# UDC-GAC/pRIblast

Measured on AMD Instinct MI355X. Metric: query RNAs/sec in `ris` step, higher is better.
Workload: dtype f64

## Files before the change

priblast_amd/csrc/gapped_args.hpp:

```cpp
#pragma once
#include <hip/hip_runtime.h>

#include <cstdint>

#include "search_device.hpp"
#include "search_kernels.hpp"

namespace prb {

struct Rec32 {
  using word = uint32_t;
  static constexpr bool kBases = true;
  static __device__ __forceinline__ word pack(int i, int j, int pred, int type, int qa, int da) {
    return (word)i | ((word)j << 7) | ((word)pred << 14) | ((word)type << 21) | ((word)qa << 24) | ((word)da << 27);
  }
  static __device__ __forceinline__ int i(word v) { return v & 0x7F; }
  static __device__ __forceinline__ int j(word v) { return (v >> 7) & 0x7F; }
  static __device__ __forceinline__ int pred(word v) { return (v >> 14) & 0x7F; }
  static __device__ __forceinline__ int type(word v) { return (v >> 21) & 7; }
  static __device__ __forceinline__ int qa(word v) { return (v >> 24) & 7; }
  static __device__ __forceinline__ int da(word v) { return (v >> 27) & 7; }
};



struct DirOrigin {
  int q_start, id_start, id_end;
  int64_t db_start;
};
__device__ __forceinline__ DirOrigin dir_origin(const HitState &h, int flag) {
  DirOrigin o;
  if (flag == 0) {
    o.q_start = h.q_sp;
    o.db_start = h.db_sp;
  } else {
    o.q_start = h.q_sp + h.q_len - 1;
    o.db_start = (int64_t)h.db_sp + h.db_len - 1;
  }
  o.id_start = h.id_start;
  o.id_end = h.id_start + h.db_len - 1;
  return o;
}


struct GapArgs {
  HitSoA in, out;
  int64_t n;
  const uint32_t *subset;
  QBatchDev qb;
  PageDev pg;
  SearchConst sc;
  ExtOpts o;
  uint8_t *overflow;
  uint8_t *tier_out;
  int tier_id;
  const uint8_t *first_flag;
  int32_t *bp_count;
  uint16_t *trace;
  const int64_t *bp_off;
  int32_t *bp_out;
  unsigned long long *next_work;
  GapResume rin, rout;
  LongTrace lt;
  double *acc_scratch = nullptr;
  int period = 0;
  int early = 0;
  int handover = 0;
};


}
```

priblast_amd/csrc/gapped_lds.hip:

```cpp
#include <algorithm>
#include <type_traits>

#include "gapped_args.hpp"
#include "search_device.hpp"
#include "search_kernels.hpp"

namespace prb {

#ifdef PRB_GAP_PROFILE
constexpr int kProfSlots = 26;
__device__ unsigned long long g_gap_prof[10 * kProfSlots];
struct GapProf {
  unsigned long long last, acc[kProfSlots];
  int cells_now = 0, cells_prev = 0;
  __device__ __forceinline__ void start() {
    for (int i = 0; i < kProfSlots; i++) acc[i] = 0;
    last = __builtin_amdgcn_s_memtime();
  }
  __device__ __forceinline__ void mark(int r) {
    const unsigned long long t = __builtin_amdgcn_s_memtime();
    acc[r] += t - last;
    last = t;
  }
  __device__ __forceinline__ void count(int r) { acc[r] += 1; }
  __device__ __forceinline__ void flush(int kind) {
    if ((threadIdx.x & 63) == 0)
      for (int i = 0; i < kProfSlots; i++) atomicAdd(&g_gap_prof[kind * kProfSlots + i], acc[i]);
  }
};
#define GP_MARK(r) prof.mark(r)
#define GP_COUNT(r) prof.count(r)
#else
struct GapProf {
  __device__ __forceinline__ void start() {}
  __device__ __forceinline__ void flush(int) {}
};
#define GP_MARK(r)
#define GP_COUNT(r)
#endif

namespace {

constexpr int kInitStage = 16;
struct Tier0 {
#ifndef PRB_T0_CAPR
#define PRB_T0_CAPR 48
#define PRB_T0_WGCU 4
#endif
#ifndef PRB_T0_ACC_GLOBAL
#define PRB_T0_ACC_GLOBAL false
#endif
  static constexpr int kG = 8, kCapD = 32, kCapR = PRB_T0_CAPR, kGroups = 32, kWavesPerSimd = PRB_T0_WGCU, kWgPerCu = PRB_T0_WGCU;
  static constexpr bool kResumable = true;
  static constexpr bool kResumes = false;
  static constexpr bool kPairSteps = true;
  static constexpr bool kAccGlobal = PRB_T0_ACC_GLOBAL;
};
#ifndef PRB_T12_ACC_GLOBAL
#define PRB_T12_ACC_GLOBAL true
#endif
#ifndef PRB_T12_WPS
#define PRB_T12_WPS (PRB_T12_ACC_GLOBAL ? 4 : 3)
#endif
#ifndef PRB_T1_CAPD
#define PRB_T1_CAPD 40
#define PRB_T1_CAPR 64
#define PRB_T1_GROUPS 32
#define PRB_T1_WGCU (PRB_T12_ACC_GLOBAL ? 4 : 3)
#endif
struct Tier1 {
  static constexpr int kG = 8, kCapD = PRB_T1_CAPD, kCapR = PRB_T1_CAPR, kGroups = PRB_T1_GROUPS, kWavesPerSimd = PRB_T12_WPS, kWgPerCu = PRB_T1_WGCU;
  static constexpr bool kResumable = true, kResumes = true;
  using From = Tier0;
  using FromRec = Rec32;
  static constexpr bool kPairSteps = false;
  static constexpr bool kAccGlobal = PRB_T12_ACC_GLOBAL;
};
struct Tier2 {
  static constexpr int kG = 16, kCapD = 64, kCapR = 120, kGroups = 16, kWavesPerSimd = PRB_T12_WPS, kWgPerCu = PRB_T12_ACC_GLOBAL ? 4 : 3;
  static constexpr bool kResumable = true, kResumes = true;
  using From = Tier1;
  using FromRec = Rec32;
  static constexpr bool kPairSteps = false;
  static constexpr bool kAccGlobal = PRB_T12_ACC_GLOBAL;
};
struct Tier3 {
  static constexpr int kG = 64, kCapD = 128, kCapR = 512, kGroups = 1, kWavesPerSimd = 4, kWgPerCu = 16;
  static constexpr bool kResumable = false, kResumes = true;
  using From = Tier2;
  using FromRec = Rec32;
  static constexpr bool kPairSteps = false;
  static constexpr bool kAccGlobal = false;
};

struct Rec32W {
  using word = uint32_t;
  static constexpr bool kBases = false;
  static __device__ __forceinline__ word pack(int i, int j, int pred, int type, int, int) {
    return (word)i | ((word)j << 8) | ((word)pred << 16) | ((word)type << 25);
  }
  static __device__ __forceinline__ int i(word v) { return v & 0xFF; }
  static __device__ __forceinline__ int j(word v) { return (v >> 8) & 0xFF; }
  static __device__ __forceinline__ int pred(word v) { return (v >> 16) & 0x1FF; }
  static __device__ __forceinline__ int type(word v) { return (v >> 25) & 7; }
// ... 644 lines not shown
        w |= (uint32_t)dpp_i32<0x141>((int)w);
        tw[c] = w;
        cells |= (cells_t)((__ballot(type1 != 0) >> gbase) & 0xFF) << (8 * c);
        GP_COUNT(11);
      }
    }
    GP_MARK(3);
#ifdef PRB_GAP_PROFILE
    prof.cells_now = kChunks <= 4 ? __popc((uint32_t)cells) : __popcll((unsigned long long)cells);
#endif
    while (cells) {
      const cells_t rest = cells & (cells - 1);
      const bool two = rest != 0 && d.nrec + 2 <= S.cap_r();
      const int b0 = kChunks <= 4 ? __builtin_ctz((uint32_t)cells) : __builtin_ctzll((unsigned long long)cells);
      if (Store::kResumable && d.nrec >= S.cap_r()) {
        d.overflow = true;
        d.resume_i0 = i_lo + b0;
        d.resume_dstart = dstart;
        break;
      }
      int b = b0;
      if (two) {
        const int b1 = kChunks <= 4 ? __builtin_ctz((uint32_t)rest) : __builtin_ctzll((unsigned long long)rest);
        if (gl >= G / 2) b = b1;
        cells = rest & (rest - 1);
      } else {
        cells = rest;
      }
      uint32_t w = tw[0];
#pragma unroll
      for (int c = 1; c < kChunks; c++) w = (b >> 3) == c ? tw[c] : w;
      const int ptype = fill_cell(i_lo + b, (int)((w >> (3 * (b & 7))) & 7), two);
      if (ptype < 0) {
        d.overflow = true;
        break;
      }
    }
    group_sync<kLds>();
    GP_MARK(3);
  } else {
    for (int i0 = i_lo; i0 <= i_hi && !d.overflow; i0 += G) {
      const int type1 = cell_type(i0 + gl);
      using mask_t = typename std::conditional<G <= 32, uint32_t, unsigned long long>::type;
      const unsigned long long tb0 = __ballot(type1 & 1), tb1 = __ballot(type1 & 2), tb2 = __ballot(type1 & 4);
      const unsigned long long anyb = tb0 | tb1 | tb2;
      mask_t vmask = G < 64 ? (mask_t)((anyb >> gbase) & ((1ull << (G & 63)) - 1)) : (mask_t)anyb;
      GP_MARK(3);
      GP_COUNT(11);
      if (Store::kResumable && d.nrec + __popcll((unsigned long long)vmask) > S.cap_r()) {
        d.overflow = true;
        d.resume_i0 = i0;
        d.resume_dstart = dstart;
        break;
      }
      while (vmask) {
        if constexpr (G == 64) {
          const int left = __popcll((unsigned long long)vmask), n = left < 4 ? left : 4;
          if (n >= 2 && d.nrec + n <= S.cap_r()) {
            fill_quad(i0, (unsigned long long)vmask, n, tb0, tb1, tb2);
            for (int t = 0; t < n; t++) vmask &= vmask - 1;
            continue;
          }
        }
        const int b = G <= 32 ? __builtin_ctz((uint32_t)vmask) : __builtin_ctzll((unsigned long long)vmask);
        vmask &= vmask - 1;
        const int ctype = (int)((tb0 >> (gbase + b)) & 1) | (int)(((tb1 >> (gbase + b)) & 1) << 1) |
                          (int)(((tb2 >> (gbase + b)) & 1) << 2);
        const int ptype = fill_cell(i0 + b, ctype, false);
        if (ptype < 0) {
          d.overflow = true;
          break;
        }
      }
      group_sync<kLds>();
      GP_MARK(3);
    }
  }
  if (d.overflow) return true;
  if (d.length - (d.min_ci + d.min_cj) >= drop) return true;
  if (!q_open && !d_open) return true;
  return false;
}

template <class Store>
__device__ __forceinline__ bool dir_step_pair(const SearchConst &sc, const SeqBases &sb, const ExtOpts &o, const HitCtx &c, int flag,
                                              const Store &S, int gl, int gbase, DirState &d, GapProf &prof) {
  constexpr int G = 8;
  using R = typename Store::R;
  static_assert(Store::kCapD <= 32, "a 32-bit mask of cells per anti-diagonal");
  constexpr int kChunks = (Store::kCapD + G - 1) / G;
  const int delta = o.delta, drop = o.drop_w_gap, min_helix = o.min_helix;
  const bool mid = d.resume_i0 != 0;
  if (!mid) {
    if (d.length >= S.cap_d()) {
      d.overflow = true;
      return true;
    }
    d.length++;
  }
  const int LA = d.length;
  const bool openA = LA < d.tq0 || LA < d.td0;
  const int curA = LA - 3 * ((LA * 171) >> 9), d2A = curA == 2 ? 0 : curA + 1;
  if (!mid) {
    if (LA > d.staged) stage_acc_regs<G, true>(sb, c, flag, delta, S, gl, gbase, d, LA);
    GP_MARK(1);
    GP_COUNT(10);
    uint64_t *row = reinterpret_cast<uint64_t *>(&S.ptab(curA, 0));
    for (int t = gl; t < S.ptab_len() / 8; t += G) row[t] = 0;
    group_sync<true>();
    if (LA - 2 > drop) {
      while (d.lo < d.nrec) {
        const auto v = S.info(d.lo);
        if (LA - R::i(v) - R::j(v) - 2 > drop) d.lo++;
        else break;
      }
    }
  }
  GP_MARK(2);
  const int dstartA = mid ? d.resume_dstart : d.nrec, loA = d.lo;
  const int i_firstA = LA - d.td0 + 1 > 1 ? LA - d.td0 + 1 : 1;
  const int i_loA = mid ? d.resume_i0 : i_firstA;
  const int i_hiA = (LA < d.tq0 ? LA : d.tq0) - 1;
  d.resume_i0 = 0;

  auto pair_type = [&](int i, int j) -> int {
    const unsigned x0 = (unsigned)S.qb(i) * 5 + S.db(j);
    int t = (int)((sc.bp_rows >> ((x0 * 3 - 15) & 63)) & 7);
    if (flag == 1) t = ((t - 1) ^ 1) + 1;
    return t;
  };
  auto helix_ok = [&](unsigned x0, unsigned x1, unsigned x2, int pt, int i, int j) -> bool {
    const unsigned p0 = (sc.pair_mask >> x0) & 1, w0 = (sc.wobble_mask >> x0) & 1;
    unsigned ahead = 1;
    if (min_helix >= 2) ahead = ((sc.pair_mask >> x1) & 1) & ~(w0 & (sc.wobble_mask >> x1));
    if (min_helix >= 3) ahead &= sc.pair_mask >> x2;
    for (int x = 3; x <= min_helix - 1; x++) ahead &= sc.pair_mask >> ((unsigned)S.qb(i + x) * 5 + S.db(j + x));
    const unsigned need = (unsigned)(pt == 0) | (w0 & (unsigned)wobble(pt));
    return (p0 & (ahead | ~need) & 1) != 0;
  };

  const int LB = LA + 1, d2B = curA == 0 ? 2 : curA - 1;
  const bool try_pair = !mid && openA && LA - (d.min_ci + d.min_cj) < drop && LA < S.cap_d() && LB <= d.staged;
  uint32_t cellsA = 0, cellsB = 0;
  int loB = loA;
  bool paired = false;
  if (try_pair) {
    if (LB - 2 > drop) {
      while (loB < dstartA) {
        const auto v = S.info(loB);
        if (LB - R::i(v) - R::j(v) - 2 > drop) loB++;
        else break;
      }
    }
    const int i_loB = LB - d.td0 + 1 > 1 ? LB - d.td0 + 1 : 1, i_hiB = (LB < d.tq0 ? LB : d.tq0) - 1;
#pragma unroll
    for (int ch = 0; ch < kChunks; ch++) {
      const int i0 = i_loA + ch * G;
      if (i0 <= i_hiB) {
        const int i = i0 + gl, j = LA - i, jc = j < 0 ? 0 : j;
        const unsigned q0 = (unsigned)S.qb(i) * 5, q1 = (unsigned)S.qb(i + 1) * 5, q2 = (unsigned)S.qb(i + 2) * 5;
        const unsigned d0 = S.db(jc), d1 = S.db(jc + 1), d2b = S.db(jc + 2), d3 = S.db(jc + 3);
        const bool okA = i <= i_hiA && helix_ok(q0 + d0, q1 + d1, q2 + d2b, S.ptab(d2A, i - 1), i, j);
        const bool okB = i >= i_loB && i <= i_hiB && helix_ok(q0 + d1, q1 + d2b, q2 + d3, S.ptab(d2B, i - 1), i, j + 1);
        cellsA |= (uint32_t)((__ballot(okA) >> gbase) & 0xFF) << (8 * ch);
        cellsB |= (uint32_t)((__ballot(okB) >> gbase) & 0xFF) << (8 * ch);
        GP_COUNT(11);
      }
    }
    if (d.nrec + __popc(cellsA) + __popc(cellsB) <= S.cap_r()) {
      paired = true;
      uint64_t *row = reinterpret_cast<uint64_t *>(&S.ptab(d2A, 0));
      for (int t = gl; t < S.ptab_len() / 8; t += G) row[t] = 0;
      group_sync<true>();
      GP_COUNT(10);
    } else {
      cellsB = 0;
    }
  } else {
#pragma unroll
    for (int ch = 0; ch < kChunks; ch++) {
      const int i0 = i_loA + ch * G;
      if (i0 <= i_hiA) {
        const int i = i0 + gl, j = LA - i, jc = j < 0 ? 0 : j;
        const unsigned x0 = (unsigned)S.qb(i) * 5 + S.db(jc), x1 = (unsigned)S.qb(i + 1) * 5 + S.db(jc + 1),
                       x2 = (unsigned)S.qb(i + 2) * 5 + S.db(jc + 2);
        const bool okA = i <= i_hiA && helix_ok(x0, x1, x2, S.ptab(d2A, i - 1), i, j);
        cellsA |= (uint32_t)((__ballot(okA) >> gbase) & 0xFF) << (8 * ch);
        GP_COUNT(11);
      }
    }
  }
  const int nA = __popc(cellsA);
  int typeA0 = 0;
  if (paired && nA != 0) {
    const int iA0 = i_loA + __builtin_ctz(cellsA);
    typeA0 = rtype_of(pair_type(iA0, LA - iA0));
  }
#ifdef PRB_GAP_PROFILE
  prof.cells_now = nA + __popc(cellsB);
#endif
  GP_MARK(3);

  auto fill_cell = [&](int ci, bool isB, bool two) -> int {
    GP_COUNT(12);
    const bool pair_mode = two, hi = pair_mode && gl >= G / 2;
    const int sub = pair_mode ? (gl & (G / 2 - 1)) : gl, stride = pair_mode ? G / 2 : G;
    const int L = LA + (isB ? 1 : 0), cur = isB ? (curA == 2 ? 0 : curA + 1) : curA, lo = isB ? loB : loA;
    const int cj = L - ci;
    const int ctype = pair_type(ci, cj);
    const int nq = S.qb(ci - 1), nd = S.db(cj - 1);
    double bte = 1000000.0;
    int bkp = lo << 3;
    const typename R::word v0 = lo + sub < dstartA ? S.info(lo + sub) : 0;
    scan_qualifying<R>(
        S, lo, dstartA, sub, stride, ci, cj, v0,
        [&](typename R::word v) -> double {
          const int ri = R::i(v), rj = R::j(v);
          const int rq = R::qa(v), rd = R::da(v);
          const bool f0 = flag == 0;
          const int rt = R::type(v);
          return loop_energy_abcd(sc, f0 ? ctype : rt, f0 ? rt : ctype, ci - ri - 1, cj - rj - 1, f0 ? nq : rq, f0 ? nd : rd,
                                  f0 ? rq : nq, f0 ? rd : nd);
        },
        bte, bkp, prof);
    GP_MARK(4);
    group_min_halves(bte, bkp, pair_mode);
    GP_MARK(5);
    if (d.nrec >= S.cap_r()) return -1;
    int bk = bkp >> 3, ptype = bkp & 7;
    const bool a_first = isB && typeA0 != 0 && lo >= dstartA;
    if (lo >= dstartA && !a_first) bk = 0;
    if (ptype == 0) ptype = a_first ? typeA0 : R::type(S.info(bk));
    const int rec = d.nrec + (hi ? 1 : 0);
    if (sub == 0) {
      S.hyb(rec) = bte;
      S.info(rec) = R::pack(ci, cj, bk, rtype_of(ctype), S.qb(ci + 1), S.db(cj + 1));
      S.ptab(cur, ci) = (uint8_t)ptype;
    }
    const double ie = S.eq(ci - 1) + S.ed(cj - 1) + bte;
    const double ie_o = dpp_f64<0x141>(ie);
    const int ci_o = dpp_i32<0x141>(ci), cj_o = dpp_i32<0x141>(cj);
    const double ie_a = hi ? ie_o : ie, ie_b = hi ? ie : ie_o;
    const int ci_a = hi ? ci_o : ci, ci_b = hi ? ci : ci_o, cj_a = hi ? cj_o : cj, cj_b = hi ? cj : cj_o;
    if (ie_a < d.min_e) {
      d.min_e = ie_a;
      d.best = d.nrec;
      d.min_ci = ci_a;
      d.min_cj = cj_a;
    }
    if (pair_mode && ie_b < d.min_e) {
      d.min_e = ie_b;
      d.best = d.nrec + 1;
      d.min_ci = ci_b;
      d.min_cj = cj_b;
    }
    d.nrec += pair_mode ? 2 : 1;
    GP_MARK(6);
    return ptype;
  };

  unsigned long long cells = (unsigned long long)cellsA | ((unsigned long long)cellsB << 32);
  while (cells) {
    const unsigned long long rest = cells & (cells - 1);
    const bool two = rest != 0 && d.nrec + 2 <= S.cap_r();
    const int b0 = __builtin_ctzll(cells);
    if (Store::kResumable && d.nrec >= S.cap_r()) {
      d.overflow = true;
      d.resume_i0 = i_loA + b0;
      d.resume_dstart = dstartA;
      break;
    }
    int b = b0;
    if (two) {
      if (gl >= G / 2) b = __builtin_ctzll(rest);
      cells = rest & (rest - 1);
    } else {
      cells = rest;
    }
    const bool isB = b >= 32;
    const int ptype = fill_cell(i_loA + (b & 31), isB, two);
    if (ptype < 0) {
      d.overflow = true;
      break;
    }
  }
  group_sync<true>();
  GP_MARK(3);
  if (d.overflow) return true;
  if (paired) {
    d.length = LA + 1;
    d.lo = loB;
    if (LB - (d.min_ci + d.min_cj) >= drop) return true;
    return !(LB < d.tq0 || LB < d.td0);
  }
  if (LA - (d.min_ci + d.min_cj) >= drop) return true;
  return !openA;
}

template <class Store> __device__ __forceinline__ DirResult dir_finish(const DirState &d, HitState &h, int flag, const Store &S) {
  DirResult r;
  r.overflow = d.overflow;
  r.best = d.min_ci != 0 ? d.best : 0;
  if (d.min_ci != 0) {
    h.e_acc = h.e_acc + S.eq(d.min_ci - 1) + S.ed(d.min_cj - 1);
    if (flag == 0) {
      h.q_sp -= d.min_ci;
      h.db_sp -= d.min_cj;
    } else {
      h.id_start -= d.min_cj;
    }
    h.q_len += d.min_ci;
    h.db_len += d.min_cj;
  }
  h.e_tot = d.min_e;
  return r;
}

struct ResumeHeader {
  DirState d;
  double acc_prev1;
  HitState h;
  int32_t flag, nleft;
};
template <class T, class Rec> constexpr size_t resume_bytes() {
  return (sizeof(ResumeHeader) + sizeof(LdsState<T, Rec>) + 63) & ~(size_t)63;
}

template <int G, class T, class Rec>
__device__ __forceinline__ void resume_dump(const GapResume &ro, const HitCtx &c, const DirState &d, int flag,
                                            const LdsStore<T, Rec> &S, int gl, int gbase) {
  int slot = -1;
  if (gl == 0) {
    slot = (int)atomicAdd(ro.count, 1u);
    if (slot >= ro.cap) slot = -1;
  }
  slot = __shfl(slot, gbase);
  if (slot < 0) return;
  uint8_t *dst = ro.pool + (size_t)slot * resume_bytes<T, Rec>();
  ResumeHeader *H = reinterpret_cast<ResumeHeader *>(dst);
  if (gl == 0) {
    H->d = d;
    H->h = c.h;
    H->flag = flag;
    H->nleft = c.nleft;
    ro.slot[c.x] = slot;
  } else if (gl == 1) {
    H->acc_prev1 = d.acc_prev;
  }
  if constexpr (!T::kAccGlobal) {
    uint32_t *w = reinterpret_cast<uint32_t *>(dst + sizeof(ResumeHeader));
    const uint32_t *src = reinterpret_cast<const uint32_t *>(&S.s);
#pragma unroll 2
    for (int t = gl; t < (int)(sizeof(LdsState<T, Rec>) / 4); t += G) w[t] = src[t];
  } else {
    LdsState<T, Rec> *o = reinterpret_cast<LdsState<T, Rec> *>(dst + sizeof(ResumeHeader));
    for (int t = gl; t < T::kCapD; t += G) {
      o->eq[t] = S.eq(t);
      o->ed[t] = S.ed(t);
    }
    for (int t = gl; t < d.nrec; t += G) {
      o->hyb[t] = S.hyb(t);
      o->info[t] = S.info(t);
    }
    uint32_t *pw = reinterpret_cast<uint32_t *>(&o->ptab[0][0]);
    const uint32_t *ps = reinterpret_cast<const uint32_t *>(&S.s.ptab[0][0]);
    for (int t = gl; t < 3 * LdsState<T, Rec>::kPtabLen / 4; t += G) pw[t] = ps[t];
  }
}

template <int G, class TS, class RecS, class Store>
__device__ __forceinline__ void resume_load(const GapResume &ri, int slot, const GapArgs &a, HitCtx &c, DirState &d, int &flag,
                                            const Store &S, int gl) {
  using R = typename Store::R;
  const uint8_t *src = ri.pool + (size_t)slot * resume_bytes<TS, RecS>();
  const ResumeHeader *H = reinterpret_cast<const ResumeHeader *>(src);
  d = H->d;
  if (G > 1 && gl == 1) d.acc_prev = H->acc_prev1;
  d.overflow = false;
  c.h = H->h;
// ... 129 lines not shown
      a.bp_count[x] = c.nleft;
      a.tier_out[x] = (uint8_t)(kResumeMark | ((c.resumed ? c.tier0 : a.tier_id) & kMarkTier));
    }
    if (!c.ovf) {
      const int64_t x = c.x;
      int tcode = a.tier_id > c.tier0 ? a.tier_id : c.tier0;
      if (a.tier_id == kWaveTier && a.lt.slot) {
        const int ls = a.lt.slot[x];
        if (ls >= 0) {
          const int c0 = a.lt.count[ls * 2], c1 = a.lt.count[ls * 2 + 1];
          if ((c0 >= 0 || (c0 == -1 && c.nleft <= kTraceCap)) && c1 >= 0) tcode = kLongTraceTier;
        }
      }
      a.tier_out[x] = (uint8_t)tcode;
      a.bp_count[x] = c.nleft | (c.nright << 16);
      const double d0 = dangle_energy_gapped(sc, h.q_sp, h.db_sp, 0, qs, c.qn, ds, a.pg.nchars);
      const double d1 = dangle_energy_gapped(sc, h.q_sp + US(h.q_len) - 1, (int64_t)h.db_sp + US(h.db_len) - 1, 1, qs, c.qn,
                                             ds, a.pg.nchars);
      double e = h.e_tot, hy = h.e_tot - h.e_acc;
      e += d0;
      e += d1;
      hy += d0;
      hy += d1;
      a.out.q_sp[x] = h.q_sp;
      a.out.db_sp[x] = h.db_sp;
      a.out.q_len[x] = h.q_len;
      a.out.db_len[x] = h.db_len;
      a.out.db_id[x] = c.id;
      a.out.db_id_start[x] = h.id_start;
      a.out.query[x] = c.query;
      a.out.e_acc[x] = h.e_acc;
      a.out.e_hyb[x] = hy;
      a.out.e_tot[x] = e;
    }
  } else if (!c.ovf) {
    int t = 0;
    const int64_t d0 = c.unsorted ? c.out0 : c.out0 + c.nleft;
    for (int u = 0; u < c.diag_len; u++)
      if (diag_pairs(sc, qs[c.diag_q + u], ds[c.diag_d + u])) {
        a.bp_out[2 * (d0 + t)] = c.diag_q + u;
        a.bp_out[2 * (d0 + t) + 1] = c.diag_d + u;
        t++;
      }
  }
}

__device__ __forceinline__ void hit_handover(const GapArgs &a, int64_t w, const HitCtx &c, int gl) {
  if (gl != 0) return;
  const int64_t x = c.x;
  const HitState &h = c.h;
  a.overflow[w] = 0;
  a.out.q_sp[x] = h.q_sp;
  a.out.db_sp[x] = h.db_sp;
  a.out.q_len[x] = h.q_len;
  a.out.db_len[x] = h.db_len;
  a.out.db_id_start[x] = h.id_start;
  a.out.e_acc[x] = h.e_acc;
  a.out.e_hyb[x] = h.e_tot - h.e_acc;
  a.out.e_tot[x] = h.e_tot;
  a.bp_count[x] = c.nleft;
  a.tier_out[x] = (uint8_t)(kHandoverMark | (a.tier_id & kMarkTier));
}

__global__ __launch_bounds__(256) void k_bp_count(HitSoA in, int64_t n, const uint32_t *__restrict__ subset, QBatchDev qb,
                                                  PageDev pg, SearchConst sc, const int32_t *__restrict__ ntrace,
                                                  int32_t *bp_count) {
  const int64_t w = (int64_t)blockIdx.x * 256 + threadIdx.x;
  if (w >= n) return;
  const int64_t x = subset ? (int64_t)subset[w] : w;
  const uint8_t *qs = qb.enc + qb.off[in.query[x]] + in.q_sp[x];
  const uint8_t *ds = pg.seqs + in.db_sp[x];
  const int len = US(in.q_len[x]);
  int c = 0;
  for (int t = 0; t < len; t++) c += diag_pairs(sc, qs[t], ds[t]);
  bp_count[w] = c + (ntrace[x] & 0xFFFF) + (int)((uint32_t)ntrace[x] >> 16);
}

template <int kMode, class T, class Rec, bool kPair>
#ifdef PRB_TIERS_VGPR128
__global__ __launch_bounds__(T::kG *T::kGroups) __attribute__((amdgpu_num_vgpr(128))) void k_gapped_lds(GapArgs a) {
#else
__global__ __launch_bounds__(T::kG *T::kGroups, T::kWavesPerSimd) void k_gapped_lds(GapArgs a) {
#endif
  static_assert(!kPair || (T::kPairSteps && T::kG == 8), "dir_step_pair");
  __shared__ LdsLive<T, Rec> lds[T::kGroups];
  constexpr int G = T::kG;
  const int gl = threadIdx.x & (G - 1);
  const int gbase = (threadIdx.x & 63) & ~(G - 1);
  const int gid = threadIdx.x / G;
  const LdsStore<T, Rec> S{lds[gid], T::kAccGlobal ? a.acc_scratch + ((size_t)blockIdx.x * T::kGroups + gid) * 2 * T::kCapD : nullptr};
  const int64_t ngroups = (int64_t)gridDim.x * T::kGroups;
  GapProf prof;
  prof.start();
  int64_t w = (int64_t)blockIdx.x * T::kGroups + gid;
  enum { kLoad, kInit, kRun, kFinished, kDone };
  int phase = w < a.n ? kLoad : kDone, flag = 0;
  const int period = a.period > 0 ? a.period : kPair ? (a.o.drop_w_gap > 1 ? (a.o.drop_w_gap + 1) / 2 : 1) : (a.o.drop_w_gap > 1 ? a.o.drop_w_gap : 1);
  int tick = 0;
  HitCtx c;
  DirState d;
  const SeqBases sb{a.qb.enc, a.qb.acc, a.qb.cond, a.pg.acc, a.pg.cond};
  while (__ballot(phase != kDone) != 0) {
    GP_MARK(14);
    if (a.early > 0 && tick != 0 && __popcll(__ballot(phase == kFinished)) >= a.early * G) tick = 0;
    if (tick == 0) {
      if (phase == kFinished) {
        DirResult r{true, 0};
        const DirOrigin og = dir_origin(c.h, flag);
        if (!d.overflow) {
          r = dir_finish(d, c.h, flag, S);
        } else {
          if constexpr (kMode == 0 && T::kResumable)
            if (a.rout.slot) resume_dump<G, T, Rec>(a.rout, c, d, flag, S, gl, gbase);
        }
        hit_dir_done<kMode, true>(a, c, flag, og, r, S, gl);
        group_sync<true>();
        GP_MARK(7);
        const bool hand = kMode == 0 && a.handover && !c.ovf && flag == 0 && !c.resumed;
        if (c.ovf || flag == 1 || hand) {
          if (hand) hit_handover(a, w, c, gl);
          else hit_store<kMode>(a, w, c, flag, gl);
          unsigned long long nw = 0;
          if (gl == 0) nw = (unsigned long long)ngroups + atomicAdd(a.next_work, 1ull);
          w = (int64_t)__shfl(nw, gbase);
          phase = w < a.n ? kLoad : kDone;
          GP_MARK(9);
        } else {
          flag = 1;
          phase = kInit;
        }
      }
      if (phase == kLoad) {
        hit_load<kMode>(a, w, c);
        flag = c.resumed ? 1 : 0;
        phase = kInit;
        if constexpr (kMode == 0 && T::kResumes) {
          const int slot = a.rin.slot ? a.rin.slot[c.x] : -1;
          if (slot >= 0) {
            resume_load<G, typename T::From, typename T::FromRec>(a.rin, slot, a, c, d, flag, S, gl);
            phase = kRun;
          }
        }
        GP_MARK(8);
      }
      if (phase == kInit) {
        dir_init<G, true>(a.sc, sb, c, flag, a.pg.seqs, a.pg.nchars, S, gl, a.o.delta, d);
        phase = kRun;
        GP_MARK(0);
      }
    }
    GP_MARK(15);
#ifdef PRB_GAP_PROFILE
    prof.cells_now = 0;
#endif
    if constexpr (kPair) {
      if (phase == kRun && dir_step_pair(a.sc, sb, a.o, c, flag, S, gl, gbase, d, prof)) phase = kFinished;
    } else {
      if (phase == kRun && dir_step<G, true>(a.sc, sb, a.o, c, flag, S, gl, gbase, d, prof)) phase = kFinished;
    }
#ifdef PRB_GAP_PROFILE
    if constexpr (G == 8) {
      auto wave_max = [](int v) {
        for (int m = 32; m >= 8; m >>= 1) {
          const int o = __shfl_xor(v, m);
          v = o > v ? o : v;
        }
        return v;
      };
      const int cn = prof.cells_now;
      prof.acc[16] += (unsigned long long)wave_max((cn + 1) / 2);
      prof.acc[17] += (unsigned long long)wave_max(cn);
      auto wave_sum = [](int v) {
        for (int m = 32; m >= 8; m >>= 1) v += __shfl_xor(v, m);
        return v;
      };
      prof.acc[18] += (unsigned long long)wave_sum(cn);
      if (tick & 1) {
        prof.acc[19] += (unsigned long long)wave_max((cn + prof.cells_prev + 1) / 2);
        prof.acc[20] += 1;
      } else {
        prof.cells_prev = cn;
      }
      prof.acc[21] += 1;
    }
#endif
    tick = tick + 1 == period ? 0 : tick + 1;
  }
  prof.flush(a.tier_id * 2 + (kMode != 0));
}

template <int kMode, bool kInLds> __global__ __launch_bounds__(64) void k_gapped_wave(GapArgs a, GapScratch scratch) {
  extern __shared__ __align__(16) uint8_t wave_smem[];
  const int gl = threadIdx.x;
  uint8_t *mine = kInLds ? wave_smem : scratch.base + (size_t)blockIdx.x * scratch.bytes_per_thread;
  HbmStore S;
  S.capd = scratch.cap_diag;
  S.capr = scratch.cap_rec;
  S.eq_ = reinterpret_cast<double *>(mine);
  S.ed_ = S.eq_ + S.capd;
  S.hyb_ = S.ed_ + S.capd;
  S.info_ = reinterpret_cast<uint64_t *>(S.hyb_ + S.capr);
  S.ptab_ = reinterpret_cast<uint8_t *>(S.info_ + S.capr);
  S.qb_ = S.ptab_ + 3 * ((size_t)S.capd + 4);
  S.db_ = S.qb_ + S.capd + 16;
  GapProf prof;
  prof.start();
  HitCtx c;
  DirState d;
  const SeqBases sb{a.qb.enc, a.qb.acc, a.qb.cond, a.pg.acc, a.pg.cond};
  for (int64_t w = blockIdx.x; w < a.n; w += gridDim.x) {
    hit_load<kMode>(a, w, c);
    int last = 0;
    bool hand = false;
    for (int flag = c.resumed ? 1 : 0; flag < 2 && !c.ovf && !hand; flag++) {
      GP_MARK(8);
      dir_init<64, false>(a.sc, sb, c, flag, a.pg.seqs, a.pg.nchars, S, gl, a.o.delta, d);
      GP_MARK(0);
      while (!dir_step<64, false>(a.sc, sb, a.o, c, flag, S, gl, 0, d, prof)) {
      }
      DirResult r{true, 0};
      const DirOrigin og = dir_origin(c.h, flag);
      if (!d.overflow) r = dir_finish(d, c.h, flag, S);
      hit_dir_done<kMode, false>(a, c, flag, og, r, S, gl);
      group_sync<false>();
      last = flag;
      hand = kMode == 0 && a.handover && !c.ovf && flag == 0 && !c.resumed;
      GP_MARK(7);
    }
    if (hand) hit_handover(a, w, c, gl);
    else hit_store<kMode>(a, w, c, last, gl);
    GP_MARK(9);
  }
  prof.flush(kWaveTier * 2 + (kMode != 0));
}

}

#ifdef PRB_GAP_PROFILE
extern "C" int prb_debug_gap_profile(unsigned long long *out, int reset) {
  if (hipDeviceSynchronize() != hipSuccess) return -1;
  if (hipMemcpyFromSymbol(out, HIP_SYMBOL(g_gap_prof), sizeof(unsigned long long) * 10 * kProfSlots) != hipSuccess) return -1;
  if (reset) {
    unsigned long long z[10 * kProfSlots] = {};
    if (hipMemcpyToSymbol(HIP_SYMBOL(g_gap_prof), z, sizeof(z)) != hipSuccess) return -1;
  }
  return 0;
}
#endif

size_t gapped_resume_bytes(int tier) {
  return tier == 0 ? resume_bytes<Tier0, Rec32>() : tier == 1 ? resume_bytes<Tier1, Rec32>() : resume_bytes<Tier2, Rec32>();
}

size_t gapped_acc_scratch_bytes() {
  if (!Tier1::kAccGlobal && !Tier0::kAccGlobal) return 0;
  const size_t t0 = (size_t)256 * Tier0::kWgPerCu * Tier0::kGroups * 2 * Tier0::kCapD * sizeof(double);
  const size_t t1 = (size_t)256 * Tier1::kWgPerCu * Tier1::kGroups * 2 * Tier1::kCapD * sizeof(double);
  const size_t t2 = (size_t)256 * Tier2::kWgPerCu * Tier2::kGroups * 2 * Tier2::kCapD * sizeof(double);
  return std::max(t0, std::max(t1, t2));
}

size_t gapped_wave_scratch_bytes(int cap_diag, int cap_rec) {
  size_t b = (size_t)cap_diag * 16 + (size_t)cap_rec * 16 + 3 * ((size_t)cap_diag + 4) + 2 * ((size_t)cap_diag + 16);
  return (b + 255) & ~(size_t)255;
}

namespace {
template <class T, class Rec> hipError_t launch_tier(const GapArgs &a, int mode, hipStream_t s) {
  const int64_t want = (a.n + T::kGroups - 1) / T::kGroups;
  const dim3 grid((unsigned)std::min<int64_t>(want, 256 * T::kWgPerCu)), blk(T::kG * T::kGroups);
  if (hipError_t e = hipMemsetAsync(a.next_work, 0, sizeof(unsigned long long), s); e != hipSuccess) return e;
  if constexpr (T::kPairSteps) {
    const char *pe = getenv("PRB_GAPPED_PAIR");
    const bool pair = !(pe && atoi(pe) == 0);
    if (pair) {
      if (mode == 0) hipLaunchKernelGGL((k_gapped_lds<0, T, Rec, true>), grid, blk, 0, s, a);
      else hipLaunchKernelGGL((k_gapped_lds<2, T, Rec, true>), grid, blk, 0, s, a);
      return hipGetLastError();
    }
  }
  size_t pad = 0;
  if (const char *pe = getenv("PRB_GAPPED_LDS_PAD")) {
    int b[4] = {0, 0, 0, 0};
    sscanf(pe, "%d,%d,%d", &b[1], &b[2], &b[3]);
    pad = (size_t)b[a.tier_id < 4 ? a.tier_id : 0];
  }
  if (mode == 0) hipLaunchKernelGGL((k_gapped_lds<0, T, Rec, false>), grid, blk, pad, s, a);
  else hipLaunchKernelGGL((k_gapped_lds<2, T, Rec, false>), grid, blk, 0, s, a);
  return hipGetLastError();
}
}

hipError_t launch_gapped_lds(const HitSoA &in, HitSoA out, int64_t n, const uint32_t *subset, const QBatchDev &qb,
                             const PageDev &pg, const SearchConst &sc, ExtOpts o, int mode, int tier, uint8_t *overflow,
                             uint8_t *tier_out, const uint8_t *first_flag, int32_t *bp_count, uint16_t *trace,
                             const int64_t *bp_off, int32_t *bp_out, unsigned long long *next_work, const GapResume &rin,
                             const GapResume &rout, hipStream_t s, int handover, double *acc_scratch) {
  if (n <= 0) return hipSuccess;
  GapArgs a{in,      out,   n,      subset, qb,        pg,         sc, o, overflow, tier_out, tier, first_flag, bp_count,
            trace,   bp_off, bp_out, next_work, rin,     rout};
  a.handover = mode == 0 ? handover : 0;
  a.acc_scratch = acc_scratch;
  if (((tier == 1 || tier == 2) && Tier1::kAccGlobal || tier == 0 && Tier0::kAccGlobal) && !acc_scratch) return hipErrorInvalidValue;
  if (const char *pe = getenv("PRB_GAPPED_PERIOD")) {
    int p[4] = {0, 0, 0, 0};
    sscanf(pe, "%d,%d,%d,%d", &p[0], &p[1], &p[2], &p[3]);
    a.period = mode == 0 && tier >= 0 && tier < 4 ? p[tier] : 0;
  }
  a.early = tier == 2 ? 2 : 0;
  if (const char *ee = getenv("PRB_GAPPED_EARLY")) {
    int k[4] = {0, 0, 0, 0};
    sscanf(ee, "%d,%d,%d,%d", &k[0], &k[1], &k[2], &k[3]);
    a.early = tier >= 0 && tier < 4 ? k[tier] : 0;
  }
  if (tier == 0) return launch_tier<Tier0, Rec32>(a, mode, s);
  if (tier == 1) return launch_tier<Tier1, Rec32>(a, mode, s);
  if (tier == 2) return launch_tier<Tier2, Rec32>(a, mode, s);
  return launch_tier<Tier3, Rec32W>(a, mode, s);
}

hipError_t launch_gapped_wave(const HitSoA &in, HitSoA out, int64_t n, const uint32_t *subset, const QBatchDev &qb,
                              const PageDev &pg, const SearchConst &sc, ExtOpts o, GapScratch scratch, int mode,
                              uint8_t *overflow, uint8_t *tier_out, const uint8_t *first_flag, int32_t *bp_count,
                              const int64_t *bp_off, int32_t *bp_out, hipStream_t s, int handover, const LongTrace &lt) {
  if (n <= 0) return hipSuccess;
  GapArgs a{in,      out,    n,      subset,  qb,      pg,      sc,      o, overflow, tier_out, kWaveTier, first_flag, bp_count,
            nullptr, bp_off, bp_out, nullptr, GapResume{nullptr, nullptr, nullptr, 0}, GapResume{nullptr, nullptr, nullptr, 0}};
  a.handover = mode == 0 ? handover : 0;
  if (mode == 0) a.lt = lt;
  const int blocks = scratch.nthreads;
  if (scratch.base == nullptr) {
    const size_t lds = scratch.bytes_per_thread;
    if (mode == 0) hipLaunchKernelGGL((k_gapped_wave<0, true>), dim3(blocks), dim3(64), lds, s, a, scratch);
    else hipLaunchKernelGGL((k_gapped_wave<2, true>), dim3(blocks), dim3(64), lds, s, a, scratch);
  } else {
    if (mode == 0) hipLaunchKernelGGL((k_gapped_wave<0, false>), dim3(blocks), dim3(64), 0, s, a, scratch);
    else hipLaunchKernelGGL((k_gapped_wave<2, false>), dim3(blocks), dim3(64), 0, s, a, scratch);
  }
  return hipGetLastError();
}

__global__ __launch_bounds__(256) void k_assign_slots(const uint32_t *__restrict__ list, int64_t n, int32_t base, int32_t *slot) {
  const int64_t p = (int64_t)blockIdx.x * 256 + threadIdx.x;
  if (p < n) slot[list[p]] = base + (int32_t)p;
}
hipError_t launch_assign_slots(const uint32_t *list, int64_t n, int32_t base, int32_t *slot, hipStream_t s) {
  if (n <= 0) return hipSuccess;
  hipLaunchKernelGGL(k_assign_slots, dim3((unsigned)((n + 255) / 256)), dim3(256), 0, s, list, n, base, slot);
  return hipGetLastError();
}

__global__ __launch_bounds__(256) void k_bp_expand(HitSoA in, int64_t n, const uint32_t *__restrict__ subset, QBatchDev qb,
                                                   PageDev pg, SearchConst sc, const uint8_t *__restrict__ first_flag,
                                                   const int32_t *__restrict__ ntrace, const uint8_t *__restrict__ tier_of,
                                                   const uint16_t *__restrict__ trace, LongTrace lt, const int64_t *__restrict__ bp_off,
                                                   int32_t *bp_out) {
  const int64_t w = (int64_t)blockIdx.x * 256 + threadIdx.x;
  if (w >= n) return;
// ... 72 lines not shown
```

Measured before the change: 7.035.

## Pool pair-step cell fills across all eight groups of a wavefront

Splits the paired anti-diagonal step into prep, fill and close phases. In the default pool mode the cells found by all eight 8-lane groups in a wavefront go into one shared work list, and 4-lane slots each take one cell from any group. This is meant to remove imbalance where some groups sit idle while others hold many cells. The running minimum-energy tracking moves to a separate reduction after the fill, and record overflow is now truncated up front. The cost is extra cross-lane shuffles, prefix sums and packed 8-bit state, plus a whole-wavefront fill that runs even when a group has finished.

```diff
diff --git a/priblast_amd/csrc/gapped_args.hpp b/priblast_amd/csrc/gapped_args.hpp
--- a/priblast_amd/csrc/gapped_args.hpp
+++ b/priblast_amd/csrc/gapped_args.hpp
@@ -65,6 +65,7 @@
   double *acc_scratch = nullptr;
   int period = 0;
   int early = 0;
+  int pool = 1;
   int handover = 0;
 };
 
diff --git a/priblast_amd/csrc/gapped_lds.hip b/priblast_amd/csrc/gapped_lds.hip
--- a/priblast_amd/csrc/gapped_lds.hip
+++ b/priblast_amd/csrc/gapped_lds.hip
@@ -8,7 +8,7 @@
 namespace prb {
 
 #ifdef PRB_GAP_PROFILE
-constexpr int kProfSlots = 26;
+constexpr int kProfSlots = 31;
 __device__ unsigned long long g_gap_prof[10 * kProfSlots];
 struct GapProf {
   unsigned long long last, acc[kProfSlots];
@@ -19,7 +19,8 @@
   }
   __device__ __forceinline__ void mark(int r) {
     const unsigned long long t = __builtin_amdgcn_s_memtime();
-    acc[r] += t - last;
+    if (t >= last) acc[r] += t - last;
+    else acc[29] += 1;
     last = t;
   }
   __device__ __forceinline__ void count(int r) { acc[r] += 1; }
@@ -830,9 +831,37 @@
   return false;
 }
 
+
+struct PairStep {
+  uint32_t cellsA, cellsB;
+  int LA, loA, loB, dstartA, i_loA, curA, typeA0, nrec;
+  bool paired;
+};
+
+__device__ __forceinline__ int nth_bit(uint32_t m, int r) {
+  int pos = 0;
+#pragma unroll
+  for (int w = 16; w >= 1; w >>= 1) {
+    const int c = __popc(m & ((1u << w) - 1));
+    if (r >= c) {
+      r -= c;
+      m >>= w;
+      pos += w;
+    }
+  }
+  return pos;
+}
+
+template <class Store> __device__ __forceinline__ int pair_type(const SearchConst &sc, const Store &S, int flag, int i, int j) {
+  const unsigned x0 = (unsigned)S.qb(i) * 5 + S.db(j);
+  int t = (int)((sc.bp_rows >> ((x0 * 3 - 15) & 63)) & 7);
+  if (flag == 1) t = ((t - 1) ^ 1) + 1;
+  return t;
+}
+
 template <class Store>
-__device__ __forceinline__ bool dir_step_pair(const SearchConst &sc, const SeqBases &sb, const ExtOpts &o, const HitCtx &c, int flag,
-                                              const Store &S, int gl, int gbase, DirState &d, GapProf &prof) {
+__device__ __forceinline__ bool pair_prep(const SearchConst &sc, const SeqBases &sb, const ExtOpts &o, const HitCtx &c, int flag,
+                                          const Store &S, int gl, int gbase, DirState &d, PairStep &p, GapProf &prof) {
   constexpr int G = 8;
   using R = typename Store::R;
   static_assert(Store::kCapD <= 32, "a 32-bit mask of cells per anti-diagonal");
@@ -871,12 +900,6 @@
   const int i_hiA = (LA < d.tq0 ? LA : d.tq0) - 1;
   d.resume_i0 = 0;
 
-  auto pair_type = [&](int i, int j) -> int {
-    const unsigned x0 = (unsigned)S.qb(i) * 5 + S.db(j);
-    int t = (int)((sc.bp_rows >> ((x0 * 3 - 15) & 63)) & 7);
-    if (flag == 1) t = ((t - 1) ^ 1) + 1;
-    return t;
-  };
   auto helix_ok = [&](unsigned x0, unsigned x1, unsigned x2, int pt, int i, int j) -> bool {
     const unsigned p0 = (sc.pair_mask >> x0) & 1, w0 = (sc.wobble_mask >> x0) & 1;
     unsigned ahead = 1;
@@ -942,107 +965,179 @@
   int typeA0 = 0;
   if (paired && nA != 0) {
     const int iA0 = i_loA + __builtin_ctz(cellsA);
-    typeA0 = rtype_of(pair_type(iA0, LA - iA0));
+    typeA0 = rtype_of(pair_type(sc, S, flag, iA0, LA - iA0));
   }
 #ifdef PRB_GAP_PROFILE
   prof.cells_now = nA + __popc(cellsB);
 #endif
+  const int room = S.cap_r() - d.nrec;
+  if (nA > room) {
+    const int keep = room > 0 ? room : 0, b = nth_bit(cellsA, keep);
+    cellsA &= (1u << b) - 1;
+    d.overflow = true;
+    if (Store::kResumable) {
+      d.resume_i0 = i_loA + b;
+      d.resume_dstart = dstartA;
+    }
+  }
+  p.cellsA = cellsA;
+  p.cellsB = cellsB;
+  p.LA = LA;
+  p.loA = loA;
+  p.loB = loB;
+  p.dstartA = dstartA;
+  p.i_loA = i_loA;
+  p.curA = curA;
+  p.typeA0 = typeA0;
+  p.nrec = d.nrec;
+  p.paired = paired;
   GP_MARK(3);
-
-  auto fill_cell = [&](int ci, bool isB, bool two) -> int {
-    GP_COUNT(12);
-    const bool pair_mode = two, hi = pair_mode && gl >= G / 2;
-    const int sub = pair_mode ? (gl & (G / 2 - 1)) : gl, stride = pair_mode ? G / 2 : G;
-    const int L = LA + (isB ? 1 : 0), cur = isB ? (curA == 2 ? 0 : curA + 1) : curA, lo = isB ? loB : loA;
-    const int cj = L - ci;
-    const int ctype = pair_type(ci, cj);
-    const int nq = S.qb(ci - 1), nd = S.db(cj - 1);
-    double bte = 1000000.0;
-    int bkp = lo << 3;
-    const typename R::word v0 = lo + sub < dstartA ? S.info(lo + sub) : 0;
-    scan_qualifying<R>(
-        S, lo, dstartA, sub, stride, ci, cj, v0,
-        [&](typename R::word v) -> double {
-          const int ri = R::i(v), rj = R::j(v);
-          const int rq = R::qa(v), rd = R::da(v);
-          const bool f0 = flag == 0;
-          const int rt = R::type(v);
-          return loop_energy_abcd(sc, f0 ? ctype : rt, f0 ? rt : ctype, ci - ri - 1, cj - rj - 1, f0 ? nq : rq, f0 ? nd : rd,
-                                  f0 ? rq : nq, f0 ? rd : nd);
-        },
-        bte, bkp, prof);
-    GP_MARK(4);
-    group_min_halves(bte, bkp, pair_mode);
-    GP_MARK(5);
-    if (d.nrec >= S.cap_r()) return -1;
-    int bk = bkp >> 3, ptype = bkp & 7;
-    const bool a_first = isB && typeA0 != 0 && lo >= dstartA;
-    if (lo >= dstartA && !a_first) bk = 0;
-    if (ptype == 0) ptype = a_first ? typeA0 : R::type(S.info(bk));
-    const int rec = d.nrec + (hi ? 1 : 0);
-    if (sub == 0) {
-      S.hyb(rec) = bte;
-      S.info(rec) = R::pack(ci, cj, bk, rtype_of(ctype), S.qb(ci + 1), S.db(cj + 1));
-      S.ptab(cur, ci) = (uint8_t)ptype;
-    }
-    const double ie = S.eq(ci - 1) + S.ed(cj - 1) + bte;
-    const double ie_o = dpp_f64<0x141>(ie);
-    const int ci_o = dpp_i32<0x141>(ci), cj_o = dpp_i32<0x141>(cj);
-    const double ie_a = hi ? ie_o : ie, ie_b = hi ? ie : ie_o;
-    const int ci_a = hi ? ci_o : ci, ci_b = hi ? ci : ci_o, cj_a = hi ? cj_o : cj, cj_b = hi ? cj : cj_o;
-    if (ie_a < d.min_e) {
-      d.min_e = ie_a;
-      d.best = d.nrec;
-      d.min_ci = ci_a;
-      d.min_cj = cj_a;
-    }
-    if (pair_mode && ie_b < d.min_e) {
-      d.min_e = ie_b;
-      d.best = d.nrec + 1;
-      d.min_ci = ci_b;
-      d.min_cj = cj_b;
-    }
-    d.nrec += pair_mode ? 2 : 1;
-    GP_MARK(6);
-    return ptype;
-  };
-
-  unsigned long long cells = (unsigned long long)cellsA | ((unsigned long long)cellsB << 32);
+  return false;
+}
+
+template <class Store>
+__device__ __forceinline__ void pair_cell(const SearchConst &sc, const Store &S, int flag, const PairStep &p, int b, int rec, int sub,
+                                          int stride, bool halves, bool act, GapProf &prof) {
+  using R = typename Store::R;
+  GP_COUNT(12);
+  const bool isB = b >= 32;
+  const int cur = isB ? (p.curA == 2 ? 0 : p.curA + 1) : p.curA;
+  const int lo = act ? (isB ? p.loB : p.loA) : 0, dstart = act ? p.dstartA : 0;
+  const int ci = act ? p.i_loA + (b & 31) : 1, cj = act ? p.LA + (isB ? 1 : 0) - ci : 1;
+  const int ctype = pair_type(sc, S, flag, ci, cj);
+  const int nq = S.qb(ci - 1), nd = S.db(cj - 1);
+  double bte = 1000000.0;
+  int bkp = lo << 3;
+  const typename R::word v0 = lo + sub < dstart ? S.info(lo + sub) : 0;
+  scan_qualifying<R>(
+      S, lo, dstart, sub, stride, ci, cj, v0,
+      [&](typename R::word v) -> double {
+        const int ri = R::i(v), rj = R::j(v);
+        const int rq = R::qa(v), rd = R::da(v);
+        const bool f0 = flag == 0;
+        const int rt = R::type(v);
+        return loop_energy_abcd(sc, f0 ? ctype : rt, f0 ? rt : ctype, ci - ri - 1, cj - rj - 1, f0 ? nq : rq, f0 ? nd : rd,
+                                f0 ? rq : nq, f0 ? rd : nd);
+      },
+      bte, bkp, prof);
+  GP_MARK(4);
+  group_min_halves(bte, bkp, halves);
+  GP_MARK(5);
+  int bk = bkp >> 3, ptype = bkp & 7;
+  const bool a_first = isB && p.typeA0 != 0 && lo >= dstart;
+  if (lo >= dstart && !a_first) bk = 0;
+  if (ptype == 0) ptype = a_first ? p.typeA0 : R::type(S.info(bk));
+  if (act && sub == 0) {
+    S.hyb(rec) = bte;
+    S.info(rec) = R::pack(ci, cj, bk, rtype_of(ctype), S.qb(ci + 1), S.db(cj + 1));
+    S.ptab(cur, ci) = (uint8_t)ptype;
+  }
+  GP_MARK(6);
+}
+
+template <class Store>
+__device__ __forceinline__ void pair_fill_group(const SearchConst &sc, const Store &S, int flag, const PairStep &p, int gl, GapProf &prof) {
+  unsigned long long cells = (unsigned long long)p.cellsA | ((unsigned long long)p.cellsB << 32);
+  int rec = p.nrec;
   while (cells) {
     const unsigned long long rest = cells & (cells - 1);
-    const bool two = rest != 0 && d.nrec + 2 <= S.cap_r();
-    const int b0 = __builtin_ctzll(cells);
-    if (Store::kResumable && d.nrec >= S.cap_r()) {
-      d.overflow = true;
-      d.resume_i0 = i_loA + b0;
-      d.resume_dstart = dstartA;
-      break;
-    }
-    int b = b0;
-    if (two) {
-      if (gl >= G / 2) b = __builtin_ctzll(rest);
-      cells = rest & (rest - 1);
-    } else {
-      cells = rest;
-    }
-    const bool isB = b >= 32;
-    const int ptype = fill_cell(i_loA + (b & 31), isB, two);
-    if (ptype < 0) {
-      d.overflow = true;
-      break;
-    }
-  }
+    const bool two = rest != 0, hi = two && gl >= 4;
+    const int b = hi ? __builtin_ctzll(rest) : __builtin_ctzll(cells);
+    pair_cell(sc, S, flag, p, b, rec + (hi ? 1 : 0), two ? (gl & 3) : gl, two ? 4 : 8, two, true, prof);
+    cells = two ? rest & (rest - 1) : rest;
+    rec += two ? 2 : 1;
+  }
+  GP_MARK(26);
   group_sync<true>();
-  GP_MARK(3);
+}
+
+template <class T, class Rec>
+__device__ __forceinline__ void pair_fill_pool(const SearchConst &sc, LdsLive<T, Rec> *wave_lds, int flag, const PairStep &p, int lane,
+                                               GapProf &prof) {
+  static_assert(T::kG == 8 && !T::kAccGlobal && T::kCapD < 255 && T::kCapR < 256, "eight groups per wavefront, state in LDS, 8-bit fields");
+  const int n = __popc(p.cellsA) + __popc(p.cellsB);
+  int incl[8];
+  int total = 0;
+#pragma unroll
+  for (int g = 0; g < 8; g++) {
+    total += __builtin_amdgcn_readlane(n, 8 * g);
+    incl[g] = total;
+  }
+  group_sync<true>();
+  const uint32_t pk0 = (uint32_t)p.LA | ((uint32_t)p.loA << 8) | ((uint32_t)p.loB << 16) | ((uint32_t)p.dstartA << 24);
+  const uint32_t pk1 = (uint32_t)p.i_loA | ((uint32_t)p.curA << 8) | ((uint32_t)p.typeA0 << 10) | ((uint32_t)flag << 13) | ((uint32_t)p.nrec << 16);
+  const int slot = lane >> 2, sub = lane & 3;
+  for (int t0 = 0; t0 < total; t0 += 16) {
+    GP_COUNT(30);
+    const int t = t0 + slot;
+    int o = 0, ex = 0;
+#pragma unroll
+    for (int g = 0; g < 7; g++) {
+      if (t >= incl[g]) {
+        o = g + 1;
+        ex = incl[g];
+      }
+    }
+    const int ob = 8 * o;
+    const uint32_t q0 = __shfl(pk0, ob), q1 = __shfl(pk1, ob), cA = __shfl(p.cellsA, ob), cB = __shfl(p.cellsB, ob);
+    PairStep po;
+    po.cellsA = cA;
+    po.cellsB = cB;
+    po.LA = q0 & 0xFF;
+    po.loA = (q0 >> 8) & 0xFF;
+    po.loB = (q0 >> 16) & 0xFF;
+    po.dstartA = q0 >> 24;
+    po.i_loA = q1 & 0xFF;
+    po.curA = (q1 >> 8) & 3;
+    po.typeA0 = (q1 >> 10) & 7;
+    po.nrec = q1 >> 16;
+    po.paired = false;
+    const int oflag = (q1 >> 13) & 1;
+    const int rank = t - ex, nA = __popc(cA);
+    const int b = rank < nA ? nth_bit(cA, rank) : 32 + nth_bit(cB, rank - nA);
+    GP_MARK(28);
+    const LdsStore<T, Rec> So{wave_lds[o], nullptr};
+    pair_cell(sc, So, oflag, po, b, po.nrec + rank, sub, 4, true, t < total, prof);
+  }
+  group_sync<true>();
+}
+
+template <class Store>
+__device__ __forceinline__ bool pair_close(const ExtOpts &o, const Store &S, int gl, DirState &d, const PairStep &p, GapProf &prof) {
+  using R = typename Store::R;
+  const int drop = o.drop_w_gap;
+  const int n = __popc(p.cellsA) + __popc(p.cellsB);
+  if (n != 0) {
+    double m = __builtin_inf();
+    int key = 0x7fffffff;
+    for (int r = gl; r < n; r += 8) {
+      const auto v = S.info(p.nrec + r);
+      const double ie = S.eq(R::i(v) - 1) + S.ed(R::j(v) - 1) + S.hyb(p.nrec + r);
+      if (ie < m) {
+        m = ie;
+        key = r;
+      }
+    }
+    group_min<8>(m, key);
+    if (m < d.min_e) {
+      const auto v = S.info(p.nrec + key);
+      d.min_e = m;
+      d.best = p.nrec + key;
+      d.min_ci = R::i(v);
+      d.min_cj = R::j(v);
+    }
+    d.nrec = p.nrec + n;
+  }
+  GP_MARK(6);
   if (d.overflow) return true;
-  if (paired) {
-    d.length = LA + 1;
-    d.lo = loB;
-    if (LB - (d.min_ci + d.min_cj) >= drop) return true;
-    return !(LB < d.tq0 || LB < d.td0);
-  }
-  if (LA - (d.min_ci + d.min_cj) >= drop) return true;
-  return !openA;
+  if (p.paired) {
+    d.length = p.LA + 1;
+    d.lo = p.loB;
+    if (p.LA + 1 - (d.min_ci + d.min_cj) >= drop) return true;
+    return !(p.LA + 1 < d.tq0 || p.LA + 1 < d.td0);
+  }
+  if (p.LA - (d.min_ci + d.min_cj) >= drop) return true;
+  return !(p.LA < d.tq0 || p.LA < d.td0);
 }
 
 template <class Store> __device__ __forceinline__ DirResult dir_finish(const DirState &d, HitState &h, int flag, const Store &S) {
@@ -1338,7 +1433,7 @@
 #else
 __global__ __launch_bounds__(T::kG *T::kGroups, T::kWavesPerSimd) void k_gapped_lds(GapArgs a) {
 #endif
-  static_assert(!kPair || (T::kPairSteps && T::kG == 8), "dir_step_pair");
+  static_assert(!kPair || (T::kPairSteps && T::kG == 8), "pair steps");
   __shared__ LdsLive<T, Rec> lds[T::kGroups];
   constexpr int G = T::kG;
   const int gl = threadIdx.x & (G - 1);
@@ -1410,7 +1505,16 @@
     prof.cells_now = 0;
 #endif
     if constexpr (kPair) {
-      if (phase == kRun && dir_step_pair(a.sc, sb, a.o, c, flag, S, gl, gbase, d, prof)) phase = kFinished;
+      const bool run = phase == kRun;
+      PairStep ps{0u, 0u, 0, 0, 0, 0, 0, 0, 0, 0, false};
+      bool fin = false;
+      if (run) fin = pair_prep(a.sc, sb, a.o, c, flag, S, gl, gbase, d, ps, prof);
+      GP_MARK(run ? 3 : 27);
+      if (a.pool) pair_fill_pool<T, Rec>(a.sc, &lds[gid & ~7], flag, ps, threadIdx.x & 63, prof);
+      else if (run) pair_fill_group(a.sc, S, flag, ps, gl, prof);
+      GP_MARK(run ? 26 : 27);
+      if (run && (fin || pair_close(a.o, S, gl, d, ps, prof))) phase = kFinished;
+      GP_MARK(run ? 6 : 27);
     } else {
       if (phase == kRun && dir_step<G, true>(a.sc, sb, a.o, c, flag, S, gl, gbase, d, prof)) phase = kFinished;
     }
@@ -1522,7 +1626,7 @@
 }
 
 namespace {
-template <class T, class Rec> hipError_t launch_tier(const GapArgs &a, int mode, hipStream_t s) {
+template <class T, class Rec> hipError_t launch_tier(GapArgs a, int mode, hipStream_t s) {
   const int64_t want = (a.n + T::kGroups - 1) / T::kGroups;
   const dim3 grid((unsigned)std::min<int64_t>(want, 256 * T::kWgPerCu)), blk(T::kG * T::kGroups);
   if (hipError_t e = hipMemsetAsync(a.next_work, 0, sizeof(unsigned long long), s); e != hipSuccess) return e;
@@ -1530,6 +1634,8 @@
     const char *pe = getenv("PRB_GAPPED_PAIR");
     const bool pair = !(pe && atoi(pe) == 0);
     if (pair) {
+      const char *pp = getenv("PRB_GAPPED_POOL");
+      a.pool = !(pp && atoi(pp) == 0);
       if (mode == 0) hipLaunchKernelGGL((k_gapped_lds<0, T, Rec, true>), grid, blk, 0, s, a);
       else hipLaunchKernelGGL((k_gapped_lds<2, T, Rec, true>), grid, blk, 0, s, a);
       return hipGetLastError();
```

Result: faster. 7.520, median of 6 (+6.9%).
